# LSaldyt/JAX_llama

Hardware: AMD Instinct MI355X
Metric: output_tokens_per_sec (higher is better)
Workload: dtype bf16; 1 GPU; model=llama3-8b, global_batch=2048, seq_len=384, prompt_len=128, gen_len=256, parallelism=dp1, mp=1

## Files before the change

jax_llama_amd/csrc/bindings.cpp:

```cpp
#include <torch/extension.h>
#include <c10/hip/HIPStream.h>

#include "kernels/launchers.h"

namespace {

using torch::Tensor;

hipStream_t stream() { return c10::hip::getCurrentHIPStream().stream(); }

void check(bool cond, const char* msg) { TORCH_CHECK(cond, "jax_llama_amd._C: ", msg); }

void check_gpu(const Tensor& t, const char* name) {
  TORCH_CHECK(t.is_cuda(), "jax_llama_amd._C: ", name, " must be a GPU tensor");
  TORCH_CHECK(t.is_contiguous(), "jax_llama_amd._C: ", name, " must be contiguous");
}

void rc(int r, const char* what) {
  TORCH_CHECK(r == 0, "jax_llama_amd._C: ", what, " failed (code ", r, ")");
}

void gemm_rc(int r, const char* what) {
  const char* why = r == -1   ? "no legal plan for this shape / tile id / epilogue / fused norm / K split"
                    : r == -3 ? "the slab workspace is missing or too small"
// ... 671 lines not shown
  const int64_t n = vals.numel();
  auto* st = reinterpret_cast<void*>(state);
  float* ov = nullptr;
  if (out_v.has_value()) {
    check_gpu(*out_v, "out_v");
    check(out_v->scalar_type() == torch::kFloat32 && out_v->numel() == out_i.numel(), "out_v");
    ov = ptr<float>(*out_v);
  }
  if (mode == 0) {
    check(out_i.numel() == n, "car_pairs argmax out shape");
  } else {
    check(mode == 1 && ov && k > 0 && n % k == 0 && out_i.numel() == n * jla::car_world(st), "car_pairs top-k shapes");
  }
  rc(jla::car_pairs(st, (int)mode, ptr<float>(vals), ptr<int32_t>(idx), (int)idx_offset, n, (int)k, ov,
                    ptr<int32_t>(out_i), stream()),
     "car_pairs");
}

}

PYBIND11_MODULE(TORCH_EXTENSION_NAME, m) {
  m.doc() = "jax_llama_amd gfx950 (MI355X) HIP kernels";
  m.attr("SKINNY_MAX_M") = SKINNY_MAX_M;
  m.attr("ARCH") = "gfx950";
  m.def("embedding", &embedding, py::arg("ids"), py::arg("table"), py::arg("out"),
        py::arg("mirror") = py::none());
  m.def("rms_scale", &rms_scale);
  m.def("rmsnorm", &rmsnorm);
  m.def("residual_add", &residual_add);
  m.def("gemm_f32", &gemm_f32);
  m.def("prefetch", &prefetch, py::arg("t"), py::arg("grid") = 128);
  m.def("linear_skinny", &linear_skinny, py::arg("x"), py::arg("w"), py::arg("n"), py::arg("k"), py::arg("out"),
        py::arg("mode"), py::arg("rms_eps"), py::arg("accumulate"), py::arg("variant"), py::arg("ws"),
        py::arg("tickets"), py::arg("mirror") = py::none(), py::arg("x_packed") = py::none(),
        py::arg("pack_out") = py::none());
  m.def("gemm", &gemm, py::arg("x"), py::arg("w"), py::arg("n"), py::arg("k"), py::arg("out"), py::arg("mode"),
        py::arg("accumulate"), py::arg("mirror") = py::none(), py::arg("ksplit") = 1, py::arg("ws") = py::none(),
        py::arg("rms_eps") = -1.0, py::arg("tile") = 0, py::arg("pack_out") = py::none(),
        py::arg("rms_ws") = py::none(), py::arg("n_body") = 0);
  m.def("gemm_tail_split", [](int64_t tiles_m, int64_t n, int64_t width, int64_t cus) {
    const int nb = jla::gemm_tail_split((int)tiles_m, (int)n, (int)width, cus > 0 ? (int)cus : jla::gemm_num_cus());
    return std::make_pair((int64_t)nb, nb > 0 ? (n - nb * width + 127) / 128 : (int64_t)0);
  }, py::arg("tiles_m"), py::arg("n"), py::arg("width"), py::arg("cus") = 0);
  m.def("gemm_plan_check", [](int64_t m, int64_t n, int64_t k, int64_t mode, bool rms, int64_t ksplit, int64_t tile,
                              bool has_rms_ws, int64_t n_body) {
    return jla::gemm_plan_check((int)m, (int)n, (int)k, (int)mode, rms, (int)ksplit, (int)tile, has_rms_ws, (int)n_body);
  }, py::arg("m"), py::arg("n"), py::arg("k"), py::arg("mode"), py::arg("rms"), py::arg("ksplit"), py::arg("tile"),
     py::arg("has_rms_ws"), py::arg("n_body") = 0);
  m.def("gemm_qkv_direct_ok", [](int64_t m, int64_t tile, int64_t k) {
    return jla::gemm_qkv_direct_ok((int)m, (int)tile, (int)k) != 0;
  });
  m.def("gemm_set_g4_default", [](int64_t on) { jla::gemm_set_g4_default((int)on); });
  m.def("gemm_set_g4_group", [](int64_t gm) { jla::gemm_set_g4_group((int)gm); });
  m.def("gemm_qkv", &gemm_qkv, py::arg("x"), py::arg("w"), py::arg("n"), py::arg("k"), py::arg("table"),
        py::arg("positions"), py::arg("kc"), py::arg("vc"), py::arg("slot"), py::arg("seq_len"), py::arg("h"),
        py::arg("hkv"), py::arg("dh"), py::arg("q"), py::arg("ksplit"), py::arg("ws"), py::arg("rms_eps") = -1.0,
        py::arg("tile") = 0, py::arg("rms_ws") = py::none());
  m.def("gemm_argmax", &gemm_argmax, py::arg("x"), py::arg("w"), py::arg("n"), py::arg("k"), py::arg("ws"),
        py::arg("rms_eps"), py::arg("idx"), py::arg("val"), py::arg("rms_ws") = py::none());
  m.def("gemm_argmax_workspace", [](int64_t m, int64_t n) { return (int64_t)jla::gemm_argmax_workspace_floats(m, n); });
  m.def("gemm_ksplit", [](int64_t m, int64_t n, int64_t k) { return jla::gemm_ksplit(m, n, k); });
  m.def("rope_kv_write", &rope_kv_write);
  m.def("attn_set_impl", [](int64_t impl, int64_t waves_target) { jla::attn_set_impl(impl, waves_target); },
        py::arg("impl"), py::arg("waves_target") = 0);
  m.def("attn_decode_splits",
        [](int64_t b, int64_t hkv, int64_t t, int64_t rep) { return jla::attn_decode_splits(b, hkv, t, rep); });
  m.def("linear_qkv", &linear_qkv, py::arg("x"), py::arg("w"), py::arg("n"), py::arg("k"), py::arg("rms_eps"),
        py::arg("table"), py::arg("positions"), py::arg("kc"), py::arg("vc"), py::arg("slot"), py::arg("seq_len"),
        py::arg("h"), py::arg("hkv"), py::arg("dh"), py::arg("q"), py::arg("variant"), py::arg("ws"), py::arg("tickets"),
        py::arg("x_packed") = py::none());
  m.def("linear_qkv_attn", &linear_qkv_attn, py::arg("x"), py::arg("w"), py::arg("n"), py::arg("k"),
        py::arg("rms_eps"), py::arg("table"), py::arg("positions"), py::arg("kc"), py::arg("vc"), py::arg("slot"),
        py::arg("h"), py::arg("hkv"), py::arg("dh"), py::arg("q"), py::arg("kv_start"), py::arg("out"),
        py::arg("out_pack"), py::arg("ws"), py::arg("tickets"), py::arg("sync"), py::arg("t_cap"), py::arg("splits"),
        py::arg("x_packed") = py::none(), py::arg("spl") = 1, py::arg("sk_ws") = py::none(),
        py::arg("sk_tk") = py::none(), py::arg("o_w") = py::none(), py::arg("o_n") = 0, py::arg("o_k") = 0,
        py::arg("o_h") = py::none(), py::arg("o_hb") = py::none(), py::arg("o_hb_pack") = py::none(),
        py::arg("tp_state") = 0);
  m.def("qkv_attn_splits", [](int64_t m, int64_t b, int64_t hkv, int64_t rep, int64_t t_cap, int64_t n, int64_t cus,
                              int64_t spl, int64_t o_groups) {
    return jla::qkv_attn_splits((int)m, (int)b, (int)hkv, (int)rep, (int)t_cap, (int)n, (int)cus, (int)spl,
                                (int)o_groups);
  }, py::arg("m"), py::arg("b"), py::arg("hkv"), py::arg("rep"), py::arg("t_cap"), py::arg("n"), py::arg("cus"),
     py::arg("spl") = 1, py::arg("o_groups") = 0);
  m.def("qkv_attn_o_groups", [](int64_t m, int64_t rep, int64_t n, int64_t k) {
    return jla::qkv_attn_o_groups((int)m, (int)rep, (int)n, (int)k);
  });
  m.def("qkv_attn_sync_ints", []() { return (int64_t)jla::qkv_attn_sync_ints(); });
  m.def("qkv_attn_set_o_nt", [](int64_t nt) { jla::qkv_attn_set_o_nt((int)nt); });
  m.def("qkv_attn_set_diag", [](int64_t d) { jla::qkv_attn_set_diag((int)d); });
  m.def("qkv_attn_set_stamps", [](c10::optional<Tensor> t) {
    if (t.has_value()) {
      check_gpu(*t, "stamps");
      check(t->scalar_type() == torch::kInt64, "stamps int64");
    }
    jla::qkv_attn_set_stamps(t.has_value() ? reinterpret_cast<unsigned long long*>(t->data_ptr()) : nullptr);
  });
  m.def("qkv_attn_occupancy", [](int64_t m, int64_t rep, int64_t spl, int64_t o_groups) {
    return jla::qkv_attn_occupancy((int)m, (int)rep, (int)spl, (int)o_groups);
  }, py::arg("m"), py::arg("rep"), py::arg("spl") = 1, py::arg("o_groups") = 0);
  m.def("attn_decode_packs", &jla::attn_decode_packs);
  m.def("skinny_workspace", &skinny_workspace);
  m.def("linear_skinny_argmax", &linear_skinny_argmax);
  m.def("gemm_tp_residual", &gemm_tp_residual, py::arg("state"), py::arg("x"), py::arg("w"), py::arg("n"), py::arg("k"),
        py::arg("h"), py::arg("hb"), py::arg("ksplit"), py::arg("ws"), py::arg("tile"));
  m.def("gemm_tp_groups", [](int64_t m, int64_t n) { return (int64_t)jla::gemm_tp_groups((int)m, (int)n); });
// ... 84 lines not shown
```

jax_llama_amd/csrc/kernels/gemm.hip:

```cpp
#include <type_traits>

#include "car.h"
#include "common.h"
#include "gemm4w.h"
#include "gemm5ws.h"
#include "gemm_plan.h"
#include "launchers.h"
#include "ring.h"

namespace jla {

constexpr int G2_BN = 256, G2_NBUF = 4, G2_GROUP_M = 8;
#ifdef JLA_GEMM_STAMPS
__device__ unsigned long long g_gemm_stamps[8192 * 8 * 6];
#endif

JLA_DEV void g2_tile_coords(int pid, int tiles_m, int tiles_n, int& tm, int& tn) {
  const int in_group = G2_GROUP_M * tiles_n;
  const int first_m = (pid / in_group) * G2_GROUP_M;
  const int gsz = min(tiles_m - first_m, G2_GROUP_M);
  tm = first_m + (pid % in_group) % gsz;
  tn = (pid % in_group) / gsz;
}

// ... 717 lines not shown
          const int row = rbase + 16 * i;
          const f32x4 v = tile_val(j, i);
          if (row < M) *reinterpret_cast<f32x4*>(static_cast<float*>(out) + (size_t)row * N + tile * 16 + 4 * q) = v;
        }
      }
    } else {
#pragma unroll
      for (int j = 0; j < NJ; ++j)
#pragma unroll
        for (int i = 0; i < 8; ++i) {
          const f32x4 v = tile_val(j, i);
          g4_stage_put<32 * PJ>(wl, 16 * i + c, 32 * j + 8 * q, u32x2{pack2bf(v[0], v[1]), pack2bf(v[2], v[3])});
        }
      bf16_t* o = static_cast<bf16_t*>(out);
      g4_stage_rows<32 * PJ>(wl, lane, [&](int r, int ch, u32x4 v) {
        const int row = mrow0 + r, col = n0 + wc * WN + 8 * ch;
        if (row < M && col < N && 8 * ch < WN) *reinterpret_cast<u32x4*>(o + (size_t)row * N + col) = v;
      });
    }
  } else {
#pragma unroll
    for (int i = 0; i < 8; ++i) {
      const int row = rbase + 16 * i;
      f32x4 hv[NJ];
#pragma unroll
      for (int j = 0; j < NJ; ++j) hv[j] = f32x4{0.f, 0.f, 0.f, 0.f};
      if constexpr (MODE == MODE_RESIDUAL) {
        if (accumulate) {
          const float* hrow = static_cast<const float*>(out) + (size_t)min(row, M - 1) * N + 4 * q;
#pragma unroll
          for (int j = 0; j < NJ; ++j)
            hv[j] = *reinterpret_cast<const f32x4*>(hrow + min((n0 >> 4) + wc * NJ + j, NTT - 1) * 16);
        }
      }
#pragma unroll
      for (int j = 0; j < NJ; ++j) hv[j] += tile_val(j, i);
#pragma unroll
      for (int j = 0; j < NJ; ++j) {
        const int tile = (n0 >> 4) + wc * NJ + j;
        if (tile >= NTT || row >= M) continue;
        const size_t idx = (size_t)row * N + tile * 16 + 4 * q;
        if constexpr (MODE == MODE_PARTIAL) {
          *reinterpret_cast<f32x4*>(static_cast<float*>(out) + (size_t)split * M * N + idx) = hv[j];
        } else {
          *reinterpret_cast<f32x4*>(static_cast<float*>(out) + idx) = hv[j];
          if (mirror)
            *reinterpret_cast<u32x2*>(mirror + idx) = u32x2{pack2bf(hv[j][0], hv[j][1]), pack2bf(hv[j][2], hv[j][3])};
        }
      }
    }
  }
}

template <int MODE, int RMSM, int NJ = 8, int DIAG = 0, bool W3 = false>
__global__ void __launch_bounds__(256, 1)
    gemm4_kernel(const bf16_t* __restrict__ x, const u32x4* __restrict__ W, void* __restrict__ out, int M, int N,
                 int K, int accumulate, int out_f32, bf16_t* __restrict__ mirror, int kc, int tiles_m, int tiles_n,
                 float rms_eps, float* __restrict__ ssq_ws, QKVArgs qa, const float* __restrict__ rms_inv,
                 int group_m) {
  constexpr bool RMS = RMSM == 1;
  __shared__ u32x4 lds[W3 ? 2 * G4_A_U4 + 3 * G4_B_U4 : 2 * G4_SLOT_U4 + 64];
  const int lane = threadIdx.x & 63;
  const int wu = __builtin_amdgcn_readfirstlane(threadIdx.x >> 6);
  const int wr = wu >> 1, wc = wu & 1;
  const int nwg = gridDim.x, orig = blockIdx.x;
  const int xcd = orig & 7, q8 = nwg >> 3, r8 = nwg & 7;
  const int wgid = (xcd < r8 ? xcd * (q8 + 1) : r8 * (q8 + 1) + (xcd - r8) * q8) + (orig >> 3);
  const int tiles = tiles_m * tiles_n;
  const int split = wgid / tiles, pid = wgid - split * tiles;
  int tm, tn;
  g4_tile_coords(pid, tiles_m, tiles_n, tm, tn, group_m);
  const int m0 = tm * G4_BM, n0 = tn * (32 * NJ);
  const int t0 = split * kc, KT = min(K >> 6, t0 + kc) - t0;

  f32x4 acc[NJ][8];
#pragma unroll
  for (int j = 0; j < NJ; ++j)
#pragma unroll
    for (int i = 0; i < 8; ++i) acc[j][i] = f32x4{0.f, 0.f, 0.f, 0.f};
  float ss[4] = {0.f, 0.f, 0.f, 0.f};
  const G4Args g{x, W, out, M, N, K, kc, tiles_m, tiles_n};
  if constexpr (NJ != 8) {
    static_assert(!RMS, "the 256 x 128 tile: precomputed statistic");
    g4n_mainloop<NJ, decltype(acc), W3>(g, lds, m0, n0, t0, KT, wu, lane, acc);
  } else {
    g4_mainloop<RMS, decltype(acc), DIAG, W3>(g, lds, m0, n0, t0, KT, wu, lane, acc, ss);
  }
  g4_epilogue<MODE, RMSM, decltype(acc), NJ>(
      acc, ss, lds, wu, lane, m0, n0, split,
      G4Epi{out, M, N, K, accumulate, out_f32, mirror, tiles_n, rms_eps, ssq_ws, rms_inv}, qa);
}

template <int MODE, int RMSM>
__global__ void __launch_bounds__(256, 1)
    gemm4p_kernel(const bf16_t* __restrict__ x, const u32x4* __restrict__ W, void* __restrict__ out, int M, int N,
                  int K, int accumulate, int out_f32, bf16_t* __restrict__ mirror, int tiles_m, int tiles_n,
                  float rms_eps, QKVArgs qa, const float* __restrict__ rms_inv, int group_m) {
  constexpr bool RMS = RMSM == 1;
  __shared__ u32x4 lds[2 * G4_SLOT_U4 + 64];
  const int lane0 = threadIdx.x & 63;
  const int wu = __builtin_amdgcn_readfirstlane(threadIdx.x >> 6);
  const int nwg = gridDim.x, orig = blockIdx.x;
  const int xcd = orig & 7, q8 = nwg >> 3, r8 = nwg & 7;
  const int wg = (xcd < r8 ? xcd * (q8 + 1) : r8 * (q8 + 1) + (xcd - r8) * q8) + (orig >> 3);
  const int tiles = tiles_m * tiles_n;
  const G4Args g{x, W, out, M, N, K, K >> 6, tiles_m, tiles_n};
  const G4Epi ep{out, M, N, K, accumulate, out_f32, mirror, tiles_n, rms_eps, nullptr, rms_inv};
  for (int pid = wg; pid < tiles; pid += nwg) {
    int tm, tn;
    g4_tile_coords(pid, tiles_m, tiles_n, tm, tn, group_m);
    const int m0 = tm * G4_BM, n0 = tn * G4_BN;
    int lane;
    asm volatile("v_mov_b32 %0, %1" : "=v"(lane) : "v"(lane0));
    f32x4 acc[8][8];
#pragma unroll
    for (int j = 0; j < 8; ++j)
#pragma unroll
      for (int i = 0; i < 8; ++i) acc[j][i] = f32x4{0.f, 0.f, 0.f, 0.f};
    float ss[4] = {0.f, 0.f, 0.f, 0.f};
    g4_mainloop<RMS>(g, lds, m0, n0, 0, K >> 6, wu, lane, acc, ss);
    g4_epilogue<MODE, RMSM>(acc, ss, lds, wu, lane, m0, n0, 0, ep, qa);
    __syncthreads();
  }
}

template <int MODE, int RMSM, int NJ>
JLA_DEV void g4t_tile(const G4Args& g, const G4Epi& ep, u32x4* lds, int m0, int n0, int wu, int lane) {
  f32x4 acc[NJ][8];
#pragma unroll
  for (int j = 0; j < NJ; ++j)
#pragma unroll
    for (int i = 0; i < 8; ++i) acc[j][i] = f32x4{0.f, 0.f, 0.f, 0.f};
  float ss[4] = {0.f, 0.f, 0.f, 0.f};
  if constexpr (NJ != 8) {
    g4n_mainloop<NJ, decltype(acc), true>(g, lds, m0, n0, 0, g.K >> 6, wu, lane, acc);
  } else {
    g4_mainloop<false, decltype(acc), 0, true>(g, lds, m0, n0, 0, g.K >> 6, wu, lane, acc, ss);
  }
  g4_epilogue<MODE, RMSM, decltype(acc), NJ>(acc, ss, lds, wu, lane, m0, n0, 0, ep, QKVArgs{});
}

JLA_DEV int g4t_remap(int orig, int nwg) {
  const int xcd = orig & 7, q8 = nwg >> 3, r8 = nwg & 7;
  return (xcd < r8 ? xcd * (q8 + 1) : r8 * (q8 + 1) + (xcd - r8) * q8) + (orig >> 3);
}

template <int MODE, int RMSM, int NJB>
__global__ void __launch_bounds__(256, 1)
    gemm4t_kernel(const bf16_t* __restrict__ x, const u32x4* __restrict__ W, void* __restrict__ out, int M, int N,
                  int K, int accumulate, int out_f32, bf16_t* __restrict__ mirror, int tiles_m, int nb, int nt,
                  float rms_eps, const float* __restrict__ rms_inv, int group_m) {
  static_assert(NJB == 6 || NJB == 8, "body tiles: 256 x 192 / 256 x 256");
  static_assert(RMSM != 1 && MODE != MODE_ARGMAX && MODE != MODE_QKV && MODE != MODE_PARTIAL, "see above");
  __shared__ u32x4 lds[2 * G4_A_U4 + 3 * G4_B_U4];
  const int lane = threadIdx.x & 63;
  const int wu = __builtin_amdgcn_readfirstlane(threadIdx.x >> 6);
  const int body = tiles_m * nb, orig = blockIdx.x;
  const G4Epi ep{out, M, N, K, accumulate, out_f32, mirror, 0, rms_eps, nullptr, rms_inv};
  int tm, tn;
  if (orig < body) {
    g4_tile_coords(g4t_remap(orig, body), tiles_m, nb, tm, tn, group_m);
    const G4Args g{x, W, out, M, N, K, K >> 6, tiles_m, nb};
    g4t_tile<MODE, RMSM, NJB>(g, ep, lds, tm * G4_BM, tn * (32 * NJB), wu, lane);
  } else {
    g4_tile_coords(g4t_remap(orig - body, tiles_m * nt), tiles_m, nt, tm, tn, group_m);
    const G4Args g{x, W, out, M, N, K, K >> 6, tiles_m, nt};
    g4t_tile<MODE, RMSM, 4>(g, ep, lds, tm * G4_BM, nb * (32 * NJB) + tn * 128, wu, lane);
  }
}

__device__ __forceinline__ float4 sum_splits(const float* __restrict__ ws, int ksplit, size_t slab4, size_t e4) {
  const float4* p = reinterpret_cast<const float4*>(ws) + e4;
  float4 v = p[0];
  for (int s0 = 1; s0 < ksplit; s0 += 8) {
    float4 q[8];
#pragma unroll
    for (int j = 0; j < 8; ++j)
      if (s0 + j < ksplit) q[j] = p[(size_t)(s0 + j) * slab4];
#pragma unroll
    for (int j = 0; j < 8; ++j)
      if (s0 + j < ksplit) {
        v.x += q[j].x;
        v.y += q[j].y;
        v.z += q[j].z;
        v.w += q[j].w;
      }
  }
  return v;
}

template <int MODE>
__global__ void __launch_bounds__(256)
    gemm_reduce_kernel(const float* __restrict__ ws, int ksplit, void* __restrict__ out, int M, int N,
                       int accumulate, int out_f32, bf16_t* __restrict__ mirror, QKVArgs qa,
                       const float* __restrict__ ssq, int K, float rms_eps) {
  const size_t t4 = (size_t)blockIdx.x * blockDim.x + threadIdx.x;
  const size_t slab4 = (size_t)M * N / 4;
  if (t4 >= (MODE == MODE_SWIGLU ? slab4 >> 1 : slab4)) return;
// ... 166 lines not shown
  const int kc = (KS + ks - 1) / ks;
  return (KS + kc - 1) / kc;
}

size_t gemm_workspace_floats(int M, int N, int K) {
  const int ks = gemm_ksplit(M, N, K);
  return ks > 1 ? (size_t)ks * M * (N + 1) : 0;
}

static int num_cus() {
  static int cus = 0;
  if (cus == 0) {
    int dev = 0;
    hipDeviceProp_t prop;
    if (hipGetDevice(&dev) == hipSuccess && hipGetDeviceProperties(&prop, dev) == hipSuccess)
      cus = prop.multiProcessorCount;
    if (cus <= 0) cus = 256;
  }
  return cus;
}
int gemm_num_cus() { return num_cus(); }

static bool g_g4_default = true;
void gemm_set_g4_default(int on) { g_g4_default = on != 0; }
int gemm_qkv_direct_ok(int M, int tile, int K) {
  const GemmPlanResult r = gemm_plan(M, 16, K, MODE_QKV, true, 1, tile, true, 0, 0, g_g4_default);
  return r.rc == 0 && !r.plan.reduce;
}
int gemm_plan_check(int M, int N, int K, int mode, int rms, int ksplit, int tile, int has_rms_ws, int n_body) {
  return gemm_plan(M, N, K, mode, rms != 0, ksplit, tile, has_rms_ws != 0, n_body, num_cus(), g_g4_default).rc;
}

struct GemmArgs {
  const bf16_t* x;
  const u32x4* w;
  void* out;
  int M, N, K, accumulate, out_f32;
  bf16_t* mirror;
  float rms_eps;
  float* ssq;
  float* rms_ws;
  QKVArgs qa;
  hipStream_t s;
};

static bool g4_row_stat(const GemmArgs& a, const GemmPlan& p, const float*& inv) {
  inv = p.norm == NORM_PRECOMPUTED ? a.rms_ws : nullptr;
  return inv == nullptr || rms_rowinv(a.x, a.rms_ws, a.M, a.K, a.rms_eps, a.s) == 0;
}

static int g_g4_group = 0;
void gemm_set_g4_group(int gm) { g_g4_group = gm; }
static int g4_group_m(int tiles_m) {
  const int gm = g_g4_group > 0 ? g_g4_group : 4;
  return gm < tiles_m ? gm : tiles_m;
}
static int g_g5_diag = 0;
void gemm5_set_diag(int d) { g_g5_diag = d; }

template <int MODE, int NJ>
static void launch_g4(const GemmArgs& a, const GemmPlan& p) {
  const int tm = (a.M + G4_BM - 1) / G4_BM, tn = (a.N + 32 * NJ - 1) / (32 * NJ);
  const int grid = tm * tn * p.ksplit, gm = g4_group_m(tm);
  const float* inv;
  if (!g4_row_stat(a, p, inv)) return;
#define JLA_G4(R, DIAG, DEEP)                                                                                       \
  gemm4_kernel<MODE, R, NJ, DIAG, DEEP><<<grid, 256, 0, a.s>>>(a.x, a.w, a.out, a.M, a.N, a.K, a.accumulate, a.out_f32, \
                                                               a.mirror, p.kc, tm, tn, a.rms_eps, a.ssq, a.qa, inv, gm)
  if constexpr (NJ != 8) {
    if (inv)
      JLA_G4(2, 0, true);
    else
      JLA_G4(0, 0, true);
  } else {
    if constexpr (MODE == MODE_STORE) {
      if (p.norm == NORM_NONE && (g_g5_diag & 192)) {
        if ((g_g5_diag & 192) == 64)
          JLA_G4(0, 1, false);
        else if ((g_g5_diag & 192) == 128)
          JLA_G4(0, 2, false);
        else
          JLA_G4(0, 3, false);
        return;
      }
    }
    if (p.norm == NORM_PRECOMPUTED) {
      if (p.deep) JLA_G4(2, 0, true); else JLA_G4(2, 0, false);
    } else if (p.norm == NORM_INLOOP) {
      if (p.deep) JLA_G4(1, 0, true); else JLA_G4(1, 0, false);
    } else {
      if (p.deep) JLA_G4(0, 0, true); else JLA_G4(0, 0, false);
    }
  }
#undef JLA_G4
}

template <int MODE>
static void launch_g4p(const GemmArgs& a, const GemmPlan& p) {
  const int tm = (a.M + G4_BM - 1) / G4_BM, tn = (a.N + G4_BN - 1) / G4_BN;
  const int grid = min(tm * tn, num_cus()), gm = g4_group_m(tm);
  const float* inv;
  if (!g4_row_stat(a, p, inv)) return;
#define JLA_G4P(R)                                                                                                  \
  gemm4p_kernel<MODE, R><<<grid, 256, 0, a.s>>>(a.x, a.w, a.out, a.M, a.N, a.K, a.accumulate, a.out_f32, a.mirror, tm, \
                                                tn, a.rms_eps, a.qa, inv, gm)
  if (p.norm == NORM_PRECOMPUTED)
    JLA_G4P(2);
  else if (p.norm == NORM_INLOOP)
    JLA_G4P(1);
  else
    JLA_G4P(0);
#undef JLA_G4P
}

template <int MODE, int NJB>
static void launch_g4t(const GemmArgs& a, const GemmPlan& p) {
  const int tm = (a.M + G4_BM - 1) / G4_BM, nt = (a.N - p.n_body * 32 * NJB + 127) / 128;
  const int grid = tm * (p.n_body + nt), gm = g4_group_m(tm);
  const float* inv;
  if (!g4_row_stat(a, p, inv)) return;
  if (inv)
    gemm4t_kernel<MODE, 2, NJB><<<grid, 256, 0, a.s>>>(a.x, a.w, a.out, a.M, a.N, a.K, a.accumulate, a.out_f32,
                                                       a.mirror, tm, p.n_body, nt, a.rms_eps, inv, gm);
  else
    gemm4t_kernel<MODE, 0, NJB><<<grid, 256, 0, a.s>>>(a.x, a.w, a.out, a.M, a.N, a.K, a.accumulate, a.out_f32,
                                                       a.mirror, tm, p.n_body, nt, a.rms_eps, nullptr, gm);
}

template <int MODE>
static void launch_g2(const GemmArgs& a, const GemmPlan& p) {
  const int cfg = p.family;
  const int bm = cfg == 1 ? 256 : 128, bn = cfg == 3 ? 128 : 256;
  const int tm = (a.M + bm - 1) / bm, tn = (a.N + bn - 1) / bn;
  const int grid = tm * tn * p.ksplit;
#define JLA_G2(WMV, LATE, R, MTV, NTV, FA, FM)                                                                     \
  gemm2_kernel<MODE, WMV, LATE, R, MTV, NTV, FA, FM><<<grid, 256 * WMV, 0, a.s>>>(                                 \
      a.x, a.w, a.out, a.M, a.N, a.K, a.accumulate, a.out_f32, a.mirror, p.kc, tm, tn, a.rms_eps, a.ssq, a.qa)
#define JLA_G2_CFG(R)                        \
  if (cfg == 2)                              \
    JLA_G2(1, false, R, 8, 4, false, 0);     \
  else if (cfg == 3)                         \
    JLA_G2(2, true, R, 4, 2, false, 0);      \
  else                                       \
    JLA_G2(2, true, R, 8, 4, true, 2)
  [[maybe_unused]] const bool rms = p.norm != NORM_NONE;
  if constexpr (MODE == MODE_QKV) {
    JLA_G2(2, true, true, 8, 4, true, 2);
  } else if constexpr (MODE == MODE_ARGMAX) {
    if (rms)
      JLA_G2(2, true, true, 8, 4, true, 2);
    else
      JLA_G2(2, true, false, 8, 4, true, 2);
  } else if constexpr (MODE == MODE_RESIDUAL) {
    JLA_G2_CFG(false);
  } else {
    if (rms) {
      JLA_G2_CFG(true);
    } else {
      JLA_G2_CFG(false);
    }
  }
#undef JLA_G2_CFG
#undef JLA_G2
}

// ... 214 lines not shown
```

jax_llama_amd/csrc/kernels/gemm4w.h:

```cpp
#pragma once
#include "common.h"

namespace jla {

constexpr int G4_BM = 256, G4_BN = 256, G4_BK = 64, G4_GROUP_M = 8;
constexpr int G4_A_U4 = G4_BM * G4_BK * 2 / 16;
constexpr int G4_B_U4 = G4_BN * G4_BK * 2 / 16;
constexpr int G4_SLOT_U4 = G4_A_U4 + G4_B_U4;

JLA_DEV void g4_tile_coords(int pid, int tiles_m, int tiles_n, int& tm, int& tn, int gm = G4_GROUP_M) {
  const int in_group = gm * tiles_n;
  const int first_m = (pid / in_group) * gm;
  const int gsz = min(tiles_m - first_m, gm);
  tm = first_m + (pid % in_group) % gsz;
  tn = (pid % in_group) / gsz;
}

JLA_DEV void g4_mfma(f32x4& acc, const u32x4& a, const u32x4& b) {
  asm volatile("v_mfma_f32_16x16x32_bf16 %0, %1, %2, %0" : "+a"(acc) : "v"(a), "v"(b));
}
JLA_DEV f32x4 g4_take(f32x4& a) {
  asm volatile("" : "+a"(a));
  return a;
}
JLA_DEV void g4_acc_fence() { asm volatile("s_nop 7\n\ts_nop 7" ::: "memory"); }

struct G4Args {
  const bf16_t* x;
  const u32x4* W;
  void* out;
  int M, N, K;
  int kc;
  int tiles_m, tiles_n;
};

template <bool RMS = false, typename Acc, int DIAG = 0, bool W3 = false>
JLA_DEV void g4_mainloop(const G4Args& g, u32x4* lds, int m0, int n0, int t0, int KT, int wu, int lane, Acc& acc,
                         float* ss = nullptr) {
  const int wr = wu >> 1, wc = wu & 1;
  const int K = g.K, KS = K >> 5, NTT = g.N >> 4;

  const char* const baseA = reinterpret_cast<const char*>(g.x + (size_t)m0 * K + (size_t)t0 * 64);
  const char* const baseB = reinterpret_cast<const char*>(g.W + ((size_t)(n0 >> 4) * KS + 2 * t0) * 64);
  unsigned offA[8], offB[8];
  const int mlast = g.M - 1 - m0;
#pragma unroll
  for (int j = 0; j < 8; ++j) {
    const int P = wu + 4 * j;
    const int row = min(8 * P + (lane >> 3), mlast);
    const int chunk = (lane & 7) ^ (4 * (P & 1) + (lane >> 4));
    offA[j] = (unsigned)row * (unsigned)K * 2u + 16u * (unsigned)chunk;
    const int f = wu + 4 * j;
    const int nt = min((n0 >> 4) + (f >> 1), NTT - 1) - (n0 >> 4);
    offB[j] = ((unsigned)nt * (unsigned)KS + (unsigned)(f & 1)) * 1024u + 16u * (unsigned)lane;
  }
  auto xslot = [&](int sl) -> u32x4* { return lds + sl * (W3 ? G4_A_U4 : G4_SLOT_U4); };
  auto wslot = [&](int sl) -> u32x4* {
    return W3 ? lds + 2 * G4_A_U4 + sl * G4_B_U4 : lds + sl * G4_SLOT_U4 + G4_A_U4;
  };
  auto dma = [&](int t, int j, int wsl) {
    if (j < 8) {
      glds16(baseA + (size_t)t * 128 + offA[j], xslot(t & 1) + (wu + 4 * j) * 64);
    } else {
      glds16(baseB + (size_t)t * 2048 + offB[j - 8], wslot(wsl) + (wu + 4 * (j - 8)) * 64);
    }
  };

  const int xrd = (wr * 128 + (lane & 15)) * 8;
  const int xc0 = (0 + (lane >> 4)) ^ ((lane >> 1) & 7), xc1 = (4 + (lane >> 4)) ^ ((lane >> 1) & 7);
  auto rd = [&](u32x4& dst, int xs, int wsl, int h, int q) {
    if (q < 8)
      dst = wslot(wsl)[((wc * 8 + q) * 2 + h) * 64 + lane];
    else
      dst = xslot(xs)[xrd + (q - 8) * 128 + (h ? xc1 : xc0)];
  };

  u32x4 w0[8], x0[8], w1[8], x1[8];

  auto substep = [&](u32x4 (&wf)[8], u32x4 (&xf)[8], u32x4 (&wn)[8], u32x4 (&xn)[8], bool do_rd, int rslot, int rw,
                     int rh, bool do_dma, int td, bool do_wdma, int tw, int tws) {
#pragma unroll
    for (int q = 0; q < 16; ++q) {
#pragma unroll
      for (int u = 0; u < 4; ++u) {
        const int e = 4 * q + u, j = e >> 3, i = e & 7;
        if constexpr (DIAG & 1)
          asm volatile("" ::"v"(wf[j]), "v"(xf[i]));
        else
          g4_mfma(acc[j][i], wf[j], xf[i]);
      }
      if (do_rd) rd(q < 8 ? wn[q] : xn[q - 8], rslot, rw, rh, q);
      if (!(DIAG & 2) && (q < 8 ? do_dma : do_wdma)) dma(q < 8 ? td : tw, q, tws);
      if constexpr (RMS) {
        if (q < 4) {
          const u32x4 f = wc ? xf[4 + q] : xf[q];
#pragma unroll
          for (int e = 0; e < 4; ++e) {
            const float lo = __uint_as_float(f[e] << 16), hi = __uint_as_float(f[e] & 0xffff0000u);
            ss[q] = fmaf(lo, lo, ss[q]);
            ss[q] = fmaf(hi, hi, ss[q]);
          }
        }
      }
    }
  };

  auto mid_barrier = [&]() {
    __builtin_amdgcn_s_waitcnt(0x0070);
    __builtin_amdgcn_s_barrier();
    asm volatile("" ::: "memory");
  };

  if constexpr (W3) {
    if (KT > 0) {
#pragma unroll
      for (int j = 0; j < 16; ++j) dma(0, j, 0);
    }
    if (KT > 1) {
#pragma unroll
      for (int j = 0; j < 16; ++j) dma(1, j, 1);
    }
    if (KT > 2) {
#pragma unroll
      for (int j = 8; j < 16; ++j) dma(2, j, 2);
      wait_vmcnt<24>();
    } else if (KT > 1) {
      wait_vmcnt<16>();
    } else {
      wait_vmcnt<0>();
    }
    __builtin_amdgcn_s_barrier();
    asm volatile("" ::: "memory");
    if (KT > 0) {
#pragma unroll
      for (int q = 0; q < 16; ++q) rd(q < 8 ? w0[q] : x0[q - 8], 0, 0, 0, q);
    }
    auto vm8_barrier = [&]() {
      __builtin_amdgcn_s_waitcnt(0x0078);
      __builtin_amdgcn_s_barrier();
      asm volatile("" ::: "memory");
    };
    int t = 0, wt = 0;
    for (; t + 3 < KT; ++t) {
      const int wn1 = wt == 2 ? 0 : wt + 1;
      substep(w0, x0, w1, x1, true, t & 1, wt, 1, false, 0, false, 0, 0);
      vm8_barrier();
      substep(w1, x1, w0, x0, true, (t + 1) & 1, wn1, 0, true, t + 2, true, t + 3, wt);
      wt = wn1;
    }
    if (t + 2 < KT) {
      const int wn1 = wt == 2 ? 0 : wt + 1;
      substep(w0, x0, w1, x1, true, t & 1, wt, 1, false, 0, false, 0, 0);
      vm8_barrier();
      substep(w1, x1, w0, x0, true, (t + 1) & 1, wn1, 0, true, t + 2, false, 0, 0);
      wt = wn1;
      ++t;
    }
    if (t + 1 < KT) {
      const int wn1 = wt == 2 ? 0 : wt + 1;
      substep(w0, x0, w1, x1, true, t & 1, wt, 1, false, 0, false, 0, 0);
      mid_barrier();
      substep(w1, x1, w0, x0, true, (t + 1) & 1, wn1, 0, false, 0, false, 0, 0);
      wt = wn1;
      ++t;
    }
    if (t < KT) {
      substep(w0, x0, w1, x1, true, t & 1, wt, 1, false, 0, false, 0, 0);
      substep(w1, x1, w0, x0, false, 0, 0, 0, false, 0, false, 0, 0);
    }
    wait_vmcnt<0>();
    g4_acc_fence();
    return;
  }

  if (KT > 0) {
#pragma unroll
    for (int j = 0; j < 16; ++j) dma(0, j, 0);
  }
  if (KT > 1) {
#pragma unroll
    for (int j = 0; j < 16; ++j) dma(1, j, 1);
    wait_vmcnt<16>();
  } else {
    wait_vmcnt<0>();
  }
  __builtin_amdgcn_s_barrier();
  asm volatile("" ::: "memory");
  if (KT > 0) {
#pragma unroll
    for (int q = 0; q < 16; ++q) rd(q < 8 ? w0[q] : x0[q - 8], 0, 0, 0, q);
  }

  int t = 0;
  for (; t + 2 < KT; ++t) {
    substep(w0, x0, w1, x1, true, t & 1, t & 1, 1, false, 0, false, 0, 0);
    mid_barrier();
    substep(w1, x1, w0, x0, true, (t + 1) & 1, (t + 1) & 1, 0, true, t + 2, true, t + 2, t & 1);
  }
  if (t + 1 < KT) {
    substep(w0, x0, w1, x1, true, t & 1, t & 1, 1, false, 0, false, 0, 0);
    mid_barrier();
    substep(w1, x1, w0, x0, true, (t + 1) & 1, (t + 1) & 1, 0, false, 0, false, 0, 0);
    ++t;
  }
  if (t < KT) {
    substep(w0, x0, w1, x1, true, t & 1, t & 1, 1, false, 0, false, 0, 0);
    substep(w1, x1, w0, x0, false, 0, 0, 0, false, 0, false, 0, 0);
  }
  g4_acc_fence();
}

template <int NJ, typename Acc, bool W3 = true>
JLA_DEV void g4n_mainloop(const G4Args& g, u32x4* lds, int m0, int n0, int t0, int KT, int wu, int lane, Acc& acc) {
  static_assert(NJ == 4 || NJ == 6 || NJ == 8, "n-tiles per wave");
  static_assert(W3, "the narrow tiles keep the weights three K-tiles deep (the two-slot form was removed in round 6)");
  constexpr int ND = NJ;
  constexpr int NQ = 8 + NJ;
  constexpr int MPS = (8 * NJ) / 16;
  const int wr = wu >> 1, wc = wu & 1;
  const int K = g.K, KS = K >> 5, NTT = g.N >> 4;
// ... 172 lines not shown
```

jax_llama_amd/csrc/kernels/gemm_plan.h:

```cpp
#pragma once

#define MODE_STORE 0
#define MODE_RESIDUAL 1
#define MODE_SWIGLU 2
#define MODE_QKV 3
#define MODE_PARTIAL 7
#define MODE_ARGMAX 8
#define MODE_TPRESID 9

namespace jla {

constexpr int G2_256_TILE = 1, G2_128_TILE = 2, G2_128N_TILE = 3;
constexpr int G4_TILE = 7, G5_TILE = 11, G5N_TILE = 12, G4P_TILE = 13, G4D_TILE = 14;
constexpr int G4N6D_TILE = 16, G4ND_TILE = 17, G4T6_TILE = 18, G4T8_TILE = 19;

enum GemmFamily {
  GEMM_NONE = 0,
  GEMM2_256x256 = 1,
  GEMM2_128x256 = 2,
  GEMM2_128x128 = 3,
  GEMM4,
  GEMM4_PERSISTENT,
  GEMM4_TAIL,
  GEMM5,
};
enum GemmNorm { NORM_NONE = 0, NORM_INLOOP = 1, NORM_PRECOMPUTED = 2 };

struct GemmPlan {
  GemmFamily family;
  int nj;
  bool deep;
  int ksplit;
  int kc;
  GemmNorm norm;
  int n_body;
  bool reduce;
};
struct GemmPlanResult {
  int rc;
  GemmPlan plan;
};

inline int gemm5_ksplit(int K, int ksplit) {
  const int KS64 = K >> 6;
  if (ksplit < 1) ksplit = 1;
  const int kc = (KS64 + ksplit - 1) / ksplit;
  return (KS64 + kc - 1) / kc;
}

inline int gemm_tail_width(int tile) { return tile == G4T6_TILE ? 192 : (tile == G4T8_TILE ? 256 : 0); }

inline int gemm_tail_split(int tiles_m, int N, int width, int cus) {
  if (tiles_m <= 0 || N <= 0 || cus <= 0 || (width != 192 && width != 256)) return 0;
  auto rounds = [&](long long wgs) { return (wgs + cus - 1) / cus; };
  auto tail_tiles = [&](int nb) { return (N - nb * width + 127) / 128; };
  auto aligned = [&](int nb) { return (tiles_m * nb) % 8 == 0 && (tiles_m * tail_tiles(nb)) % 8 == 0; };
  long long best = rounds((long long)tiles_m * ((N + width - 1) / width)) * width * 16;
  int best_nb = 0;
  for (int nb = (N - 1) / width; nb >= 1; --nb) {
    const long long cost =
        rounds((long long)tiles_m * nb) * width * 16 + rounds((long long)tiles_m * tail_tiles(nb)) * 128 * 17;
    if (cost < best || (best_nb != 0 && cost == best && aligned(nb) && !aligned(best_nb))) {
      best = cost;
      best_nb = nb;
    }
  }
  return best_nb;
}

inline GemmPlanResult gemm_plan(int M, int N, int K, int mode, bool rms, int ksplit, int tile, bool has_rms_ws,
                                int n_body, int cus, bool g4_default) {
  GemmPlan p{};
  const auto fail = [](int rc) { return GemmPlanResult{rc, GemmPlan{}}; };
  const bool k64 = (K & 63) == 0;
  const bool caller_mode = mode == MODE_STORE || mode == MODE_RESIDUAL || mode == MODE_SWIGLU || mode == MODE_QKV ||
                           mode == MODE_TPRESID;

  if (tile == G5_TILE || tile == G5N_TILE) {
    if (mode == MODE_ARGMAX || (rms && (mode == MODE_RESIDUAL || mode == MODE_TPRESID))) return fail(-1);
    if (K <= 0 || !k64 || (N & 15) || M <= 0) return fail(-1);
    if (mode == MODE_SWIGLU && (N & 31)) return fail(-1);
    if (!caller_mode) return fail(-1);
    p.family = GEMM5;
    p.nj = tile == G5_TILE ? 4 : 2;
    p.ksplit = gemm5_ksplit(K, ksplit);
    p.kc = ((K >> 6) + p.ksplit - 1) / p.ksplit;
    p.norm = rms ? NORM_INLOOP : NORM_NONE;
    p.reduce = true;
    return {0, p};
  }

  if (tile == G4ND_TILE && (!k64 || (mode == MODE_QKV && ksplit <= 1) || mode == MODE_ARGMAX ||
                            (rms && mode != MODE_RESIDUAL && (ksplit > 1 || !has_rms_ws))))
    return fail(-1);
  if (M <= 0) return {0, p};
  if (K <= 0 || (N & 15) || (K & 31)) return fail(-1);
  if (mode == MODE_SWIGLU && (N & 31)) return fail(-1);
  if (rms && mode == MODE_RESIDUAL) return fail(-5);
  const int KS = K >> 5;
  p.kc = (KS + (ksplit < 1 ? 1 : ksplit) - 1) / (ksplit < 1 ? 1 : ksplit);
  p.ksplit = (KS + p.kc - 1) / p.kc;
  const bool split = p.ksplit > 1;
  if (mode == MODE_TPRESID && (!split || rms)) return fail(-1);
  const int lmode = split ? MODE_PARTIAL : mode;
  p.reduce = split;

  const bool tail = tile == G4T6_TILE || tile == G4T8_TILE;
  if (tail) {
    p.family = GEMM4_TAIL;
    p.nj = tile == G4T6_TILE ? 6 : 8;
  } else if (tile == G4ND_TILE) {
    p.family = GEMM4, p.nj = 4, p.deep = true;
  } else if (tile == G4N6D_TILE && k64 && lmode != MODE_ARGMAX) {
    p.family = GEMM4, p.nj = 6, p.deep = true;
  } else if (k64 && (tile == G4_TILE || tile == G4P_TILE || tile == G4D_TILE || (tile == 0 && g4_default && M > 128))) {
    const bool persist = tile == G4P_TILE || (lmode == MODE_RESIDUAL && tile == 0 && M >= 4096);
    p.family = persist && !split && lmode != MODE_ARGMAX ? GEMM4_PERSISTENT : GEMM4;
    p.nj = 8, p.deep = tile == G4D_TILE;
  } else if (mode == MODE_ARGMAX) {
    p.family = GEMM2_256x256;
  } else {
    p.family = tile >= G2_256_TILE && tile <= G2_128N_TILE ? (GemmFamily)tile
                                                           : (M <= 128 ? GEMM2_128x256 : GEMM2_256x256);
  }
  const bool g4 = p.family == GEMM4 || p.family == GEMM4_PERSISTENT || p.family == GEMM4_TAIL;
  if (g4) p.kc = ((K >> 6) + p.ksplit - 1) / p.ksplit;

  if (mode == MODE_QKV && !split &&
      !(rms && ((p.family == GEMM2_256x256 && (tile == 0 || tile == G2_256_TILE)) || p.family == GEMM4 ||
                p.family == GEMM4_PERSISTENT)))
    return fail(-1);
  if ((tile == G4ND_TILE || tile == G4N6D_TILE) && rms && (split || !has_rms_ws)) return fail(-6);
  if (tail) {
    if (!k64 || split || (mode != MODE_STORE && mode != MODE_RESIDUAL && mode != MODE_SWIGLU)) return fail(-1);
    if (rms && !has_rms_ws) return fail(-6);
    const int wb = gemm_tail_width(tile);
    p.n_body = n_body > 0 ? n_body : gemm_tail_split((M + 255) / 256, N, wb, cus);
    if (p.n_body <= 0 || (long long)p.n_body * wb >= N) return fail(-7);
  }
  if (mode == MODE_ARGMAX ? split : !caller_mode) return fail(-1);

  if (rms) p.norm = g4 && !split && has_rms_ws ? NORM_PRECOMPUTED : NORM_INLOOP;
  return {0, p};
}

}
```

Baseline: 43730 tokens/s.

## Add deep-X GEMM pipeline with triple-buffered activations for large-M projections

Adds a new DEEP==2 variant of the 256x256 gemm4 mainloop in which the activation (X) tile is triple-buffered in LDS and the weight tile is double-buffered, the mirror image of the existing deep-W variant. The plan auto-selects it for large-M unsplit residual (persistent) GEMMs and for precomputed-norm store/swiglu/qkv GEMMs above size thresholds. The aim is to hide activation load latency where M is large and X traffic dominates, at the cost of a larger LDS footprint. It also moves tile-coordinate and XCD-remap helpers into a shared host/device header and exposes a tile-order inspection binding.

```diff
diff --git a/jax_llama_amd/csrc/bindings.cpp b/jax_llama_amd/csrc/bindings.cpp
--- a/jax_llama_amd/csrc/bindings.cpp
+++ b/jax_llama_amd/csrc/bindings.cpp
@@ -747,6 +747,24 @@
   });
   m.def("gemm_set_g4_default", [](int64_t on) { jla::gemm_set_g4_default((int)on); });
   m.def("gemm_set_g4_group", [](int64_t gm) { jla::gemm_set_g4_group((int)gm); });
+  m.def("gemm_tile_order", [](int64_t tiles_m, int64_t tiles_n, int64_t params, int64_t workgroups) {
+    const int tiles = (int)(tiles_m * tiles_n), nwg = (int)workgroups;
+    check(tiles_m > 0 && tiles_n > 0 && nwg > 0 && tiles_m * tiles_n < (1ll << 31), "gemm_tile_order: sizes");
+    Tensor r = torch::empty({(int64_t)tiles, 2}, torch::dtype(torch::kInt64));
+    int64_t* o = r.data_ptr<int64_t>();
+    int i = 0;
+    for (int orig = 0; orig < nwg; ++orig)
+      for (int pid = jla::g4_xcd_remap(orig, nwg); pid < tiles; pid += nwg, ++i) {
+        int tm, tn;
+        jla::g4_tile_coords(pid, (int)tiles_m, (int)tiles_n, tm, tn, (int)params);
+        check(i < tiles, "gemm_tile_order: more visits than tiles");
+        o[2 * i] = tm, o[2 * i + 1] = tn;
+      }
+    check(i == tiles, "gemm_tile_order: fewer visits than tiles");
+    return r;
+  }, py::arg("tiles_m"), py::arg("tiles_n"), py::arg("params"), py::arg("workgroups"));
+  m.def("gemm_tile_order_params", []() { return std::vector<int64_t>{1, 2, 4, 8, 16}; });
+  m.def("gemm_tile_order_default", []() { return (int64_t)jla::G4_GROUP_DEFAULT; });
   m.def("gemm_qkv", &gemm_qkv, py::arg("x"), py::arg("w"), py::arg("n"), py::arg("k"), py::arg("table"),
         py::arg("positions"), py::arg("kc"), py::arg("vc"), py::arg("slot"), py::arg("seq_len"), py::arg("h"),
         py::arg("hkv"), py::arg("dh"), py::arg("q"), py::arg("ksplit"), py::arg("ws"), py::arg("rms_eps") = -1.0,
diff --git a/jax_llama_amd/csrc/kernels/gemm.hip b/jax_llama_amd/csrc/kernels/gemm.hip
--- a/jax_llama_amd/csrc/kernels/gemm.hip
+++ b/jax_llama_amd/csrc/kernels/gemm.hip
@@ -793,20 +793,19 @@
   }
 }
 
-template <int MODE, int RMSM, int NJ = 8, int DIAG = 0, bool W3 = false>
+template <int MODE, int RMSM, int NJ = 8, int DIAG = 0, int DEEP = 0>
 __global__ void __launch_bounds__(256, 1)
     gemm4_kernel(const bf16_t* __restrict__ x, const u32x4* __restrict__ W, void* __restrict__ out, int M, int N,
                  int K, int accumulate, int out_f32, bf16_t* __restrict__ mirror, int kc, int tiles_m, int tiles_n,
                  float rms_eps, float* __restrict__ ssq_ws, QKVArgs qa, const float* __restrict__ rms_inv,
                  int group_m) {
   constexpr bool RMS = RMSM == 1;
-  __shared__ u32x4 lds[W3 ? 2 * G4_A_U4 + 3 * G4_B_U4 : 2 * G4_SLOT_U4 + 64];
+  static_assert(DEEP != 2 || NJ == 8, "deep x: the 256 x 256 tile only");
+  __shared__ u32x4 lds[DEEP ? 2 * G4_A_U4 + 3 * G4_B_U4 : 2 * G4_SLOT_U4 + 64];
   const int lane = threadIdx.x & 63;
   const int wu = __builtin_amdgcn_readfirstlane(threadIdx.x >> 6);
   const int wr = wu >> 1, wc = wu & 1;
-  const int nwg = gridDim.x, orig = blockIdx.x;
-  const int xcd = orig & 7, q8 = nwg >> 3, r8 = nwg & 7;
-  const int wgid = (xcd < r8 ? xcd * (q8 + 1) : r8 * (q8 + 1) + (xcd - r8) * q8) + (orig >> 3);
+  const int wgid = g4_xcd_remap(blockIdx.x, gridDim.x);
   const int tiles = tiles_m * tiles_n;
   const int split = wgid / tiles, pid = wgid - split * tiles;
   int tm, tn;
@@ -823,27 +822,26 @@
   const G4Args g{x, W, out, M, N, K, kc, tiles_m, tiles_n};
   if constexpr (NJ != 8) {
     static_assert(!RMS, "the 256 x 128 tile: precomputed statistic");
-    g4n_mainloop<NJ, decltype(acc), W3>(g, lds, m0, n0, t0, KT, wu, lane, acc);
+    g4n_mainloop<NJ, decltype(acc), DEEP == 1>(g, lds, m0, n0, t0, KT, wu, lane, acc);
   } else {
-    g4_mainloop<RMS, decltype(acc), DIAG, W3>(g, lds, m0, n0, t0, KT, wu, lane, acc, ss);
+    g4_mainloop<RMS, decltype(acc), DIAG, DEEP>(g, lds, m0, n0, t0, KT, wu, lane, acc, ss);
   }
   g4_epilogue<MODE, RMSM, decltype(acc), NJ>(
       acc, ss, lds, wu, lane, m0, n0, split,
       G4Epi{out, M, N, K, accumulate, out_f32, mirror, tiles_n, rms_eps, ssq_ws, rms_inv}, qa);
 }
 
-template <int MODE, int RMSM>
+template <int MODE, int RMSM, int DEEP = 0>
 __global__ void __launch_bounds__(256, 1)
     gemm4p_kernel(const bf16_t* __restrict__ x, const u32x4* __restrict__ W, void* __restrict__ out, int M, int N,
                   int K, int accumulate, int out_f32, bf16_t* __restrict__ mirror, int tiles_m, int tiles_n,
                   float rms_eps, QKVArgs qa, const float* __restrict__ rms_inv, int group_m) {
   constexpr bool RMS = RMSM == 1;
-  __shared__ u32x4 lds[2 * G4_SLOT_U4 + 64];
+  __shared__ u32x4 lds[DEEP ? 2 * G4_A_U4 + 3 * G4_B_U4 : 2 * G4_SLOT_U4 + 64];
   const int lane0 = threadIdx.x & 63;
   const int wu = __builtin_amdgcn_readfirstlane(threadIdx.x >> 6);
-  const int nwg = gridDim.x, orig = blockIdx.x;
-  const int xcd = orig & 7, q8 = nwg >> 3, r8 = nwg & 7;
-  const int wg = (xcd < r8 ? xcd * (q8 + 1) : r8 * (q8 + 1) + (xcd - r8) * q8) + (orig >> 3);
+  const int nwg = gridDim.x;
+  const int wg = g4_xcd_remap(blockIdx.x, nwg);
   const int tiles = tiles_m * tiles_n;
   const G4Args g{x, W, out, M, N, K, K >> 6, tiles_m, tiles_n};
   const G4Epi ep{out, M, N, K, accumulate, out_f32, mirror, tiles_n, rms_eps, nullptr, rms_inv};
@@ -859,7 +857,7 @@
 #pragma unroll
       for (int i = 0; i < 8; ++i) acc[j][i] = f32x4{0.f, 0.f, 0.f, 0.f};
     float ss[4] = {0.f, 0.f, 0.f, 0.f};
-    g4_mainloop<RMS>(g, lds, m0, n0, 0, K >> 6, wu, lane, acc, ss);
+    g4_mainloop<RMS, decltype(acc), 0, DEEP>(g, lds, m0, n0, 0, K >> 6, wu, lane, acc, ss);
     g4_epilogue<MODE, RMSM>(acc, ss, lds, wu, lane, m0, n0, 0, ep, qa);
     __syncthreads();
   }
@@ -881,10 +879,7 @@
   g4_epilogue<MODE, RMSM, decltype(acc), NJ>(acc, ss, lds, wu, lane, m0, n0, 0, ep, QKVArgs{});
 }
 
-JLA_DEV int g4t_remap(int orig, int nwg) {
-  const int xcd = orig & 7, q8 = nwg >> 3, r8 = nwg & 7;
-  return (xcd < r8 ? xcd * (q8 + 1) : r8 * (q8 + 1) + (xcd - r8) * q8) + (orig >> 3);
-}
+JLA_DEV int g4t_remap(int orig, int nwg) { return g4_xcd_remap(orig, nwg); }
 
 template <int MODE, int RMSM, int NJB>
 __global__ void __launch_bounds__(256, 1)
@@ -1157,7 +1152,7 @@
 static int g_g4_group = 0;
 void gemm_set_g4_group(int gm) { g_g4_group = gm; }
 static int g4_group_m(int tiles_m) {
-  const int gm = g_g4_group > 0 ? g_g4_group : 4;
+  const int gm = g_g4_group > 0 ? g_g4_group : G4_GROUP_DEFAULT;
   return gm < tiles_m ? gm : tiles_m;
 }
 static int g_g5_diag = 0;
@@ -1174,27 +1169,33 @@
                                                                a.mirror, p.kc, tm, tn, a.rms_eps, a.ssq, a.qa, inv, gm)
   if constexpr (NJ != 8) {
     if (inv)
-      JLA_G4(2, 0, true);
+      JLA_G4(2, 0, 1);
     else
-      JLA_G4(0, 0, true);
+      JLA_G4(0, 0, 1);
   } else {
+    if constexpr (MODE == MODE_STORE || MODE == MODE_SWIGLU || MODE == MODE_QKV) {
+      if (p.deepx) {
+        JLA_G4(2, 0, 2);
+        return;
+      }
+    }
     if constexpr (MODE == MODE_STORE) {
       if (p.norm == NORM_NONE && (g_g5_diag & 192)) {
         if ((g_g5_diag & 192) == 64)
-          JLA_G4(0, 1, false);
+          JLA_G4(0, 1, 0);
         else if ((g_g5_diag & 192) == 128)
-          JLA_G4(0, 2, false);
+          JLA_G4(0, 2, 0);
         else
-          JLA_G4(0, 3, false);
+          JLA_G4(0, 3, 0);
         return;
       }
     }
     if (p.norm == NORM_PRECOMPUTED) {
-      if (p.deep) JLA_G4(2, 0, true); else JLA_G4(2, 0, false);
+      if (p.deep) JLA_G4(2, 0, 1); else JLA_G4(2, 0, 0);
     } else if (p.norm == NORM_INLOOP) {
-      if (p.deep) JLA_G4(1, 0, true); else JLA_G4(1, 0, false);
+      if (p.deep) JLA_G4(1, 0, 1); else JLA_G4(1, 0, 0);
     } else {
-      if (p.deep) JLA_G4(0, 0, true); else JLA_G4(0, 0, false);
+      if (p.deep) JLA_G4(0, 0, 1); else JLA_G4(0, 0, 0);
     }
   }
 #undef JLA_G4
@@ -1206,9 +1207,14 @@
   const int grid = min(tm * tn, num_cus()), gm = g4_group_m(tm);
   const float* inv;
   if (!g4_row_stat(a, p, inv)) return;
-#define JLA_G4P(R)                                                                                                  \
-  gemm4p_kernel<MODE, R><<<grid, 256, 0, a.s>>>(a.x, a.w, a.out, a.M, a.N, a.K, a.accumulate, a.out_f32, a.mirror, tm, \
-                                                tn, a.rms_eps, a.qa, inv, gm)
+#define JLA_G4P_ARGS a.x, a.w, a.out, a.M, a.N, a.K, a.accumulate, a.out_f32, a.mirror, tm, tn, a.rms_eps, a.qa, inv, gm
+#define JLA_G4P(R) gemm4p_kernel<MODE, R><<<grid, 256, 0, a.s>>>(JLA_G4P_ARGS)
+  if constexpr (MODE == MODE_RESIDUAL) {
+    if (p.deepx) {
+      gemm4p_kernel<MODE, 0, 2><<<grid, 256, 0, a.s>>>(JLA_G4P_ARGS);
+      return;
+    }
+  }
   if (p.norm == NORM_PRECOMPUTED)
     JLA_G4P(2);
   else if (p.norm == NORM_INLOOP)
@@ -1216,6 +1222,7 @@
   else
     JLA_G4P(0);
 #undef JLA_G4P
+#undef JLA_G4P_ARGS
 }
 
 template <int MODE, int NJB>
diff --git a/jax_llama_amd/csrc/kernels/gemm4w.h b/jax_llama_amd/csrc/kernels/gemm4w.h
--- a/jax_llama_amd/csrc/kernels/gemm4w.h
+++ b/jax_llama_amd/csrc/kernels/gemm4w.h
@@ -1,20 +1,14 @@
 #pragma once
 #include "common.h"
+#include "gemm_plan.h"
 
 namespace jla {
 
-constexpr int G4_BM = 256, G4_BN = 256, G4_BK = 64, G4_GROUP_M = 8;
+constexpr int G4_BM = 256, G4_BN = 256, G4_BK = 64;
 constexpr int G4_A_U4 = G4_BM * G4_BK * 2 / 16;
 constexpr int G4_B_U4 = G4_BN * G4_BK * 2 / 16;
 constexpr int G4_SLOT_U4 = G4_A_U4 + G4_B_U4;
 
-JLA_DEV void g4_tile_coords(int pid, int tiles_m, int tiles_n, int& tm, int& tn, int gm = G4_GROUP_M) {
-  const int in_group = gm * tiles_n;
-  const int first_m = (pid / in_group) * gm;
-  const int gsz = min(tiles_m - first_m, gm);
-  tm = first_m + (pid % in_group) % gsz;
-  tn = (pid % in_group) / gsz;
-}
 
 JLA_DEV void g4_mfma(f32x4& acc, const u32x4& a, const u32x4& b) {
   asm volatile("v_mfma_f32_16x16x32_bf16 %0, %1, %2, %0" : "+a"(acc) : "v"(a), "v"(b));
@@ -34,7 +28,7 @@
   int tiles_m, tiles_n;
 };
 
-template <bool RMS = false, typename Acc, int DIAG = 0, bool W3 = false>
+template <bool RMS = false, typename Acc, int DIAG = 0, int DEEP = 0>
 JLA_DEV void g4_mainloop(const G4Args& g, u32x4* lds, int m0, int n0, int t0, int KT, int wu, int lane, Acc& acc,
                          float* ss = nullptr) {
   const int wr = wu >> 1, wc = wu & 1;
@@ -54,15 +48,16 @@
     const int nt = min((n0 >> 4) + (f >> 1), NTT - 1) - (n0 >> 4);
     offB[j] = ((unsigned)nt * (unsigned)KS + (unsigned)(f & 1)) * 1024u + 16u * (unsigned)lane;
   }
-  auto xslot = [&](int sl) -> u32x4* { return lds + sl * (W3 ? G4_A_U4 : G4_SLOT_U4); };
+  constexpr bool W3 = DEEP == 1, X3 = DEEP == 2;
+  auto xslot = [&](int sl) -> u32x4* { return lds + sl * (DEEP ? G4_A_U4 : G4_SLOT_U4); };
   auto wslot = [&](int sl) -> u32x4* {
-    return W3 ? lds + 2 * G4_A_U4 + sl * G4_B_U4 : lds + sl * G4_SLOT_U4 + G4_A_U4;
-  };
-  auto dma = [&](int t, int j, int wsl) {
+    return DEEP ? lds + (X3 ? 3 : 2) * G4_A_U4 + sl * G4_B_U4 : lds + sl * G4_SLOT_U4 + G4_A_U4;
+  };
+  auto dma = [&](int t, int j, int dsl) {
     if (j < 8) {
-      glds16(baseA + (size_t)t * 128 + offA[j], xslot(t & 1) + (wu + 4 * j) * 64);
+      glds16(baseA + (size_t)t * 128 + offA[j], xslot(X3 ? dsl : (t & 1)) + (wu + 4 * j) * 64);
     } else {
-      glds16(baseB + (size_t)t * 2048 + offB[j - 8], wslot(wsl) + (wu + 4 * (j - 8)) * 64);
+      glds16(baseB + (size_t)t * 2048 + offB[j - 8], wslot(X3 ? (t & 1) : dsl) + (wu + 4 * (j - 8)) * 64);
     }
   };
 
@@ -90,7 +85,7 @@
           g4_mfma(acc[j][i], wf[j], xf[i]);
       }
       if (do_rd) rd(q < 8 ? wn[q] : xn[q - 8], rslot, rw, rh, q);
-      if (!(DIAG & 2) && (q < 8 ? do_dma : do_wdma)) dma(q < 8 ? td : tw, q, tws);
+      if (!(DIAG & 2) && (q < 8 ? do_dma : do_wdma)) dma(q < 8 ? td : tw, X3 ? (q ^ 8) : q, tws);
       if constexpr (RMS) {
         if (q < 4) {
           const u32x4 f = wc ? xf[4 + q] : xf[q];
@@ -111,7 +106,7 @@
     asm volatile("" ::: "memory");
   };
 
-  if constexpr (W3) {
+  if constexpr (DEEP != 0) {
     if (KT > 0) {
 #pragma unroll
       for (int j = 0; j < 16; ++j) dma(0, j, 0);
@@ -122,7 +117,7 @@
     }
     if (KT > 2) {
 #pragma unroll
-      for (int j = 8; j < 16; ++j) dma(2, j, 2);
+      for (int j = 0; j < 8; ++j) dma(2, X3 ? j : j + 8, 2);
       wait_vmcnt<24>();
     } else if (KT > 1) {
       wait_vmcnt<16>();
@@ -140,32 +135,34 @@
       __builtin_amdgcn_s_barrier();
       asm volatile("" ::: "memory");
     };
-    int t = 0, wt = 0;
+    auto xs = [&](int t, int d) { return X3 ? d : (t & 1); };
+    auto ws = [&](int t, int d) { return X3 ? (t & 1) : d; };
+    int t = 0, dt = 0;
     for (; t + 3 < KT; ++t) {
-      const int wn1 = wt == 2 ? 0 : wt + 1;
-      substep(w0, x0, w1, x1, true, t & 1, wt, 1, false, 0, false, 0, 0);
+      const int dn1 = dt == 2 ? 0 : dt + 1;
+      substep(w0, x0, w1, x1, true, xs(t, dt), ws(t, dt), 1, false, 0, false, 0, 0);
       vm8_barrier();
-      substep(w1, x1, w0, x0, true, (t + 1) & 1, wn1, 0, true, t + 2, true, t + 3, wt);
-      wt = wn1;
+      substep(w1, x1, w0, x0, true, xs(t + 1, dn1), ws(t + 1, dn1), 0, true, t + 2, true, t + 3, dt);
+      dt = dn1;
     }
     if (t + 2 < KT) {
-      const int wn1 = wt == 2 ? 0 : wt + 1;
-      substep(w0, x0, w1, x1, true, t & 1, wt, 1, false, 0, false, 0, 0);
+      const int dn1 = dt == 2 ? 0 : dt + 1;
+      substep(w0, x0, w1, x1, true, xs(t, dt), ws(t, dt), 1, false, 0, false, 0, 0);
       vm8_barrier();
-      substep(w1, x1, w0, x0, true, (t + 1) & 1, wn1, 0, true, t + 2, false, 0, 0);
-      wt = wn1;
+      substep(w1, x1, w0, x0, true, xs(t + 1, dn1), ws(t + 1, dn1), 0, true, t + 2, false, 0, 0);
+      dt = dn1;
       ++t;
     }
     if (t + 1 < KT) {
-      const int wn1 = wt == 2 ? 0 : wt + 1;
-      substep(w0, x0, w1, x1, true, t & 1, wt, 1, false, 0, false, 0, 0);
+      const int dn1 = dt == 2 ? 0 : dt + 1;
+      substep(w0, x0, w1, x1, true, xs(t, dt), ws(t, dt), 1, false, 0, false, 0, 0);
       mid_barrier();
-      substep(w1, x1, w0, x0, true, (t + 1) & 1, wn1, 0, false, 0, false, 0, 0);
-      wt = wn1;
+      substep(w1, x1, w0, x0, true, xs(t + 1, dn1), ws(t + 1, dn1), 0, false, 0, false, 0, 0);
+      dt = dn1;
       ++t;
     }
     if (t < KT) {
-      substep(w0, x0, w1, x1, true, t & 1, wt, 1, false, 0, false, 0, 0);
+      substep(w0, x0, w1, x1, true, xs(t, dt), ws(t, dt), 1, false, 0, false, 0, 0);
       substep(w1, x1, w0, x0, false, 0, 0, 0, false, 0, false, 0, 0);
     }
     wait_vmcnt<0>();
diff --git a/jax_llama_amd/csrc/kernels/gemm_plan.h b/jax_llama_amd/csrc/kernels/gemm_plan.h
--- a/jax_llama_amd/csrc/kernels/gemm_plan.h
+++ b/jax_llama_amd/csrc/kernels/gemm_plan.h
@@ -8,11 +8,30 @@
 #define MODE_ARGMAX 8
 #define MODE_TPRESID 9
 
+#if defined(__HIPCC__)
+#define JLA_PLAN_HD __host__ __device__ inline
+#else
+#define JLA_PLAN_HD inline
+#endif
+
 namespace jla {
+
+JLA_PLAN_HD void g4_tile_coords(int pid, int tiles_m, int tiles_n, int& tm, int& tn, int gm) {
+  const int in_group = gm * tiles_n;
+  const int first_m = (pid / in_group) * gm;
+  const int gsz = tiles_m - first_m < gm ? tiles_m - first_m : gm;
+  tm = first_m + (pid % in_group) % gsz;
+  tn = (pid % in_group) / gsz;
+}
+
+JLA_PLAN_HD int g4_xcd_remap(int orig, int nwg) {
+  const int xcd = orig & 7, q8 = nwg >> 3, r8 = nwg & 7;
+  return (xcd < r8 ? xcd * (q8 + 1) : r8 * (q8 + 1) + (xcd - r8) * q8) + (orig >> 3);
+}
 
 constexpr int G2_256_TILE = 1, G2_128_TILE = 2, G2_128N_TILE = 3;
 constexpr int G4_TILE = 7, G5_TILE = 11, G5N_TILE = 12, G4P_TILE = 13, G4D_TILE = 14;
-constexpr int G4N6D_TILE = 16, G4ND_TILE = 17, G4T6_TILE = 18, G4T8_TILE = 19;
+constexpr int G4N6D_TILE = 16, G4ND_TILE = 17, G4T6_TILE = 18, G4T8_TILE = 19, G4X_TILE = 21;
 
 enum GemmFamily {
   GEMM_NONE = 0,
@@ -30,6 +49,7 @@
   GemmFamily family;
   int nj;
   bool deep;
+  bool deepx;
   int ksplit;
   int kc;
   GemmNorm norm;
@@ -47,6 +67,9 @@
   const int kc = (KS64 + ksplit - 1) / ksplit;
   return (KS64 + kc - 1) / kc;
 }
+
+constexpr int G4_GROUP_DEFAULT = 4;
+constexpr int G4X_MIN_M = 32768, G4X_RESID_MIN_M = 8192;
 
 inline int gemm_tail_width(int tile) { return tile == G4T6_TILE ? 192 : (tile == G4T8_TILE ? 256 : 0); }
 
@@ -109,6 +132,18 @@
   if (tail) {
     p.family = GEMM4_TAIL;
     p.nj = tile == G4T6_TILE ? 6 : 8;
+  } else if (tile == G4X_TILE) {
+    if (!k64 || split) return fail(-1);
+    if (mode == MODE_RESIDUAL) {
+      p.family = GEMM4_PERSISTENT;
+    } else if (mode == MODE_STORE || mode == MODE_SWIGLU || mode == MODE_QKV) {
+      if (!rms) return fail(-1);
+      if (!has_rms_ws) return fail(-6);
+      p.family = GEMM4;
+    } else {
+      return fail(-1);
+    }
+    p.nj = 8, p.deepx = true;
   } else if (tile == G4ND_TILE) {
     p.family = GEMM4, p.nj = 4, p.deep = true;
   } else if (tile == G4N6D_TILE && k64 && lmode != MODE_ARGMAX) {
@@ -141,6 +176,11 @@
   if (mode == MODE_ARGMAX ? split : !caller_mode) return fail(-1);
 
   if (rms) p.norm = g4 && !split && has_rms_ws ? NORM_PRECOMPUTED : NORM_INLOOP;
+  if (tile == 0 && g4 && p.nj == 8 && !split &&
+      ((M >= G4X_RESID_MIN_M && p.family == GEMM4_PERSISTENT && mode == MODE_RESIDUAL) ||
+       (M >= G4X_MIN_M && p.family == GEMM4 && p.norm == NORM_PRECOMPUTED &&
+        (mode == MODE_STORE || mode == MODE_SWIGLU || mode == MODE_QKV))))
+    p.deepx = true;
   return {0, p};
 }
 
```

New measurement: 43850 tokens/s, median of 6. No clear change (+0.3%).
